# liuzhenboo/Stereo-Visual-Odometry

Hardware: AMD Instinct MI355X
Metric: stereo frames/sec on KITTI-00 1241x376; LK-kernel achieved HBM GB/s vs peak (higher is better)
Workload: dtype u8; 1 GPU; S0 synthetic KITTI-like stereo sequence 1241x376 (config #2 stand-in), FAST+LK track_mode LK_stereof2f_pnp, batched frame pairs (256 per step, 4 distinct chunks cycled), frames resident in HBM for `value`; `m1` (--full) = host-resident frames, H2D included; pairs_ok_last_step=256, parallelism=1 GPU

## Files before the change

stereo-visual-odometry_amd/binding.py:

```python
import ctypes as C
import os
import subprocess

import numpy as np

_HERE = os.path.dirname(os.path.abspath(__file__))
_LIB = None

MEM_HOST, MEM_DEVICE = 0, 1

KP_DTYPE = np.dtype([("x", "<f4"), ("y", "<f4"), ("size", "<f4"), ("angle", "<f4"),
                     ("response", "<f4"), ("octave", "<i4"), ("class_id", "<i4")])


class SvoError(RuntimeError):
    pass


class Config(C.Structure):
    _fields_ = [("width", C.c_int32), ("height", C.c_int32), ("max_keypoints", C.c_int32),
                ("max_batch", C.c_int32), ("num_slots", C.c_int32), ("fast_threshold", C.c_int32),
                ("num_features_tracking", C.c_int32), ("iterations", C.c_int32),
                ("reproj_err", C.c_float), ("confidence", C.c_float),
                ("feature_match_error", C.c_double), ("inlier_rate", C.c_double),
# ... 246 lines not shown
        return [(names[i].decode(), float(ms[i])) for i in range(n)]

    def _img(self, img, shape=None):
        shape = shape or (self.height, self.width)
        assert tuple(img.shape) == tuple(shape), (tuple(img.shape), shape)
        if isinstance(img, np.ndarray):
            assert img.dtype == np.uint8 and img.strides[1] == 1
            return C.c_void_p(img.ctypes.data), int(img.strides[0]), MEM_HOST
        assert img.element_size() == 1 and img.stride(1) == 1
        return C.c_void_p(img.data_ptr()), int(img.stride(0)), (MEM_DEVICE if img.is_cuda else MEM_HOST)

    def fast_detect(self, img, threshold=20, nonmax=True, cap=None):
        cap = cap or self.cfg.max_keypoints
        p, pitch, mem = self._img(img)
        out = np.zeros(cap, dtype=KP_DTYPE)
        n = C.c_int(0)
        self._check(self.lib.svo_fast_detect(self.h, p, pitch, mem, int(threshold), int(bool(nonmax)),
                                             C.c_void_p(out.ctypes.data), cap, C.byref(n)))
        return out[:n.value].copy()

    def build_pyramid(self, slot, img):
        p, pitch, mem = self._img(img)
        self._check(self.lib.svo_build_pyramid(self.h, int(slot), p, pitch, mem))

    def read_pyramid_level(self, slot, level):
        w, h = C.c_int(0), C.c_int(0)
        self._check(self.lib.svo_read_pyramid_level(self.h, slot, level, None, 0, MEM_HOST,
                                                    C.byref(w), C.byref(h)))
        out = np.zeros((h.value, w.value), np.uint8)
        self._check(self.lib.svo_read_pyramid_level(self.h, slot, level, C.c_void_p(out.ctypes.data),
                                                    w.value, MEM_HOST, C.byref(w), C.byref(h)))
        return out

    def lk_track(self, slot_prev, slot_next, pts):
        if isinstance(pts, np.ndarray):
            pts = np.ascontiguousarray(pts, np.float32).reshape(-1, 2)
            n = pts.shape[0]
            out = np.zeros((n, 2), np.float32)
            st = np.zeros(n, np.uint8)
        else:
            import torch
            n = pts.shape[0]
            out = torch.zeros((n, 2), dtype=torch.float32, device=pts.device)
            st = torch.zeros(n, dtype=torch.uint8, device=pts.device)
            self._order_in(st)
        pi, mem = _ptr(pts)
        po, _ = _ptr(out)
        ps, _ = _ptr(st)
        self._check(self.lib.svo_lk_track(self.h, slot_prev, slot_next, pi, n, po, ps, mem))
        if mem == MEM_DEVICE:
            self._order_out(st)
        return out, st

    def circular_match(self, slots, t1_left):
        if isinstance(t1_left, np.ndarray):
            t1_left = np.ascontiguousarray(t1_left, np.float32).reshape(-1, 2)
            n = t1_left.shape[0]
            outs = [np.zeros((max(n, 1), 2), np.float32) for _ in range(4)]
        else:
            import torch
            n = t1_left.shape[0]
            outs = [torch.zeros((max(n, 1), 2), dtype=torch.float32, device=t1_left.device) for _ in range(4)]
            self._order_in(outs[0])
        pi, mem = _ptr(t1_left)
        m = C.c_int(0)
        self._check(self.lib.svo_circular_match(self.h, *[int(s) for s in slots], pi, n,
# ... 374 lines not shown
```

stereo-visual-odometry_amd/csrc/fast.hip:

```cpp
#include "svo_device.h"
#include "svo_kernels.h"

namespace svo {

constexpr int kTileW = 64, kTileH = 16, kHalo = 4;
constexpr int kRawW = kTileW + 2 * kHalo;
constexpr int kRawH = kTileH + 2 * kHalo;
constexpr int kScW = kTileW + 2;
constexpr int kScH = kTileH + 2;

__device__ __forceinline__ void load_circle(const uint8_t *c, int d[16], int v)
{
    constexpr int P = kRawW;
    d[0] = v - c[3 * P];       d[1] = v - c[3 * P + 1];   d[2] = v - c[2 * P + 2];   d[3] = v - c[P + 3];
    d[4] = v - c[3];           d[5] = v - c[-P + 3];      d[6] = v - c[-2 * P + 2];  d[7] = v - c[-3 * P + 1];
    d[8] = v - c[-3 * P];      d[9] = v - c[-3 * P - 1];  d[10] = v - c[-2 * P - 2]; d[11] = v - c[-P - 3];
    d[12] = v - c[-3];         d[13] = v - c[P - 3];      d[14] = v - c[2 * P - 2];  d[15] = v - c[3 * P - 1];
}

__device__ __forceinline__ bool has_arc9(unsigned m16)
{
    unsigned m = m16 | (m16 << 16);
    unsigned a = m & (m >> 1);
    unsigned b = a & (a >> 2);
    unsigned c = b & (b >> 4);
    unsigned e = c & (m >> 8);
    return (e & 0xFFFFu) != 0;
}

__device__ __forceinline__ bool fast_arc(const uint8_t *c, int thr)
{
    int d[16];
    load_circle(c, d, c[0]);
    unsigned dark = 0, bright = 0;
#pragma unroll
    for (int k = 0; k < 16; k++) {
        dark |= (unsigned)(d[k] > thr) << k;
        bright |= (unsigned)(d[k] < -thr) << k;
// ... 112 lines not shown
            if (c0 + c1 + c2 + c3) {
                int base = 0;
                if (lane == 0) base = atomicAdd(&n_cand, c0 + c1 + c2 + c3);
                base = __builtin_amdgcn_readfirstlane(base);
                const int pos = sy * kScW + sxb;
                if (m4 & 1u) cand[base + __popcll(b0 & lt)] = (uint16_t)pos;
                if (m4 & 2u) cand[base + c0 + __popcll(b1 & lt)] = (uint16_t)(pos + 1);
                if (m4 & 4u) cand[base + c0 + c1 + __popcll(b2 & lt)] = (uint16_t)(pos + 2);
                if (m4 & 8u) cand[base + c0 + c1 + c2 + __popcll(b3 & lt)] = (uint16_t)(pos + 3);
            }
        }
    }
    __syncthreads();
    const int nc = n_cand;
    for (int i0 = 0; i0 < nc; i0 += 256) {
        const int i = i0 + tid;
        const int pos = i < nc ? cand[i] : 0;
        const int sy = pos / kScW, sx = pos - sy * kScW;
        const bool corner = i < nc && fast_arc(&raw[(sy + kHalo - 1) * kRawW + sx + kHalo - 1], a.thr);
        if (a.nms) list_push(corner, pos, corners, &n_corner);
        else if (corner) sc[pos] = 1;
    }
    __syncthreads();
    if (a.nms) {
        const int nk = n_corner;
        for (int i = tid; i < nk; i += 256) {
            const int pos = corners[i];
            const int sy = pos / kScW, sx = pos - sy * kScW;
            sc[pos] = (uint8_t)fast_corner_score(&raw[(sy + kHalo - 1) * kRawW + sx + kHalo - 1], a.thr);
        }
        __syncthreads();
    }

#pragma unroll
    for (int j = 0; j < kTileH / 4; j++) {
        int ly = threadIdx.y + 4 * j, lx = threadIdx.x;
        int gx = x0 + lx, gy = y0 + ly;
        const uint8_t *p = &sc[(ly + 1) * kScW + lx + 1];
        int s = p[0];
        if (a.nms && s) {
            bool keep = s > p[-1] && s > p[1] && s > p[-kScW - 1] && s > p[-kScW] && s > p[-kScW + 1] &&
                        s > p[kScW - 1] && s > p[kScW] && s > p[kScW + 1];
            if (!keep) s = 0;
        }
        bool inimg = gx < a.w && gy < a.h;
        if (!inimg) s = 0;
        unsigned long long m = __ballot(s != 0);
        if (inimg) score[(int64_t)gy * a.spitch + gx] = (uint8_t)s;
        if (threadIdx.x == 0 && m && gy < a.h) atomicAdd(&rowcount[gy], __popcll(m));
    }
}

__global__ __launch_bounds__(256) void fast_emit_kernel(FastArgs a)
{
    const int b = blockIdx.y;
    const int y = blockIdx.x * 4 + (threadIdx.x >> 6);
    const int lane = threadIdx.x & 63;
    if (y >= a.h) return;
    const uint8_t *score = a.score + (int64_t)b * a.score_stride + (int64_t)y * a.spitch;
    const int *rowcount = a.rowcount + (int64_t)b * a.rowcount_stride;
    int mine = rowcount[y];
    bool last = (y == a.h - 1);
    if (mine == 0 && !last) return;
    int part = 0;
    for (int r = lane; r < y; r += 64) part += rowcount[r];
    int off = wave_sum_i32(part);
    if (last && lane == 0) a.n_out[b] = off + mine;
    if (mine == 0) return;
    float2 *xy = a.kp_xy + (int64_t)b * a.kp_stride;
    float *resp = a.kp_resp + (int64_t)b * a.kp_stride;
    for (int x = lane; x < ((a.w + 63) & ~63); x += 64) {
        int s = x < a.w ? score[x] : 0;
        unsigned long long m = __ballot(s != 0);
        if (s) {
            int idx = off + __popcll(m & ((1ull << lane) - 1ull));
            if (idx < a.cap) {
                xy[idx] = make_float2((float)x, (float)y);
                resp[idx] = a.nms ? (float)s : 0.f;
            }
        }
        off += __popcll(m);
    }
}

__global__ __launch_bounds__(1024) void fast_keep_strongest_kernel(FastArgs a, int keep)
{
    __shared__ int hist[256];
    __shared__ int wave_eq[16], wave_kp[16];
    __shared__ int s_t, s_need_eq, s_eq_base, s_out_base;
    const int b = blockIdx.x, tid = threadIdx.x, lane = tid & 63, wv = tid >> 6;
    const int n = a.n_out[b];
    if (n <= keep || n > a.cap) return;
    float2 *xy = a.kp_xy + (int64_t)b * a.kp_stride;
    float *resp = a.kp_resp + (int64_t)b * a.kp_stride;
    if (tid < 256) hist[tid] = 0;
    __syncthreads();
    for (int i = tid; i < n; i += 1024) atomicAdd(&hist[min(255, max(0, (int)resp[i]))], 1);
    __syncthreads();
    if (tid == 0) {
        int above = 0, t = 255;
        for (; t > 0; t--) {
            if (above + hist[t] >= keep) break;
            above += hist[t];
        }
        s_t = t; s_need_eq = keep - above; s_eq_base = 0; s_out_base = 0;
    }
    __syncthreads();
    const int t = s_t, need_eq = s_need_eq;
    for (int start = 0; start < n; start += 1024) {
        const int i = start + tid;
        const bool in = i < n;
        const float2 p = in ? xy[i] : make_float2(0.f, 0.f);
        const float r = in ? resp[i] : 0.f;
        const int ri = (int)r;
// ... 178 lines not shown
```

stereo-visual-odometry_amd/csrc/pipeline.hip:

```cpp
#include <cstring>
#include "svo_ctx.h"

namespace svo {

void timing_mark(svo_ctx *ctx, const char *name)
{
    if (!ctx->timing) return;
    if (ctx->ev_used >= 16384) return;
    if (ctx->ev_used == ctx->ev_pool.size()) {
        hipEvent_t ev = nullptr;
        if (hipEventCreate(&ev) != hipSuccess) return;
        ctx->ev_pool.push_back(ev);
    }
    hipEvent_t ev = ctx->ev_pool[ctx->ev_used++];
    (void)hipEventRecord(ev, ctx->stream);
    ctx->marks.emplace_back(name, ev);
}
static inline void mark(svo_ctx *ctx, const char *name) { timing_mark(ctx, name); }

static const char *kTMatch = "orb_match";
static const char *kT0 = "start", *kTPyr = "pyramid", *kTFast = "fast", *kTLk = "lk", *kTCompact = "compact",
                  *kTTri = "triangulate", *kTPnp = "pnp", *kTFin = "finalize";

static int ingest_frames(svo_ctx *ctx, const uint8_t *L, const uint8_t *R, int pitch, int64_t frame_stride,
// ... 138 lines not shown

static int run_pairs(svo_ctx *ctx, int n_pairs, int fp0, int fc0, int fstep, const double *pose0_host,
                     svo_step_result *results_dev, const StreamStep *ss = nullptr)
{
    const PyrGeom &g = ctx->geom;
    const int cap = ctx->cfg.max_keypoints;
    if (ctx->cfg.track_mode == SVO_MODE_ORB) {
        if (ctx->back_pending) {
            SVO_HIP(hipStreamWaitEvent(ctx->stream, ctx->ev_back, 0));
            ctx->back_pending = false;
        }
        orb_match_pairs(ctx, n_pairs, fp0, fc0, fstep, ctx->stream);
        mark(ctx, kTMatch);
        const SnapSpec snap{(const int *)ctx->orb_n, (const int *)ctx->orb_overflow, fp0, fc0, fstep, 2};
        launch_triangulate_batch(ctx, n_pairs, cap, ctx->cmp[0], ctx->cmp[1], ctx->m_out, 0, &snap);
        mark(ctx, kTTri);
        return run_back(ctx, n_pairs, pose0_host, results_dev, false, ss);
    }
    auto S = [&](int slot) { return ctx->bslots + (size_t)slot * g.slot_bytes; };
    LkArgs a{};
    a.g = g; a.ncalls = 4;
    a.slot_stride = (int64_t)fstep * 2 * g.slot_bytes;
    a.prev[0] = S(2 * fp0);     a.next[0] = S(2 * fp0 + 1);
    a.prev[1] = S(2 * fp0 + 1); a.next[1] = S(2 * fc0 + 1);
    a.prev[2] = S(2 * fc0 + 1); a.next[2] = S(2 * fc0);
    a.prev[3] = S(2 * fc0);     a.next[3] = S(2 * fp0);
    a.pts_in = ctx->kp_xy + (size_t)fp0 * cap; a.pts_stride = (int64_t)fstep * cap;
    a.n_pts = ctx->kp_n + fp0;
    a.n_fixed = 0; a.cap = cap;
    for (int i = 0; i < 4; i++) { a.pts_out[i] = ctx->pts_out[i]; a.status[i] = ctx->status[i]; }
    a.keep = ctx->keep;
    a.match_err = ctx->cfg.feature_match_error; a.match_err_f = (float)ctx->cfg.feature_match_error;
    a.accum = ctx->cfg.lk_accum;
    launch_lk(a, n_pairs, cap, ctx->stream);
    mark(ctx, kTLk);
    if (ctx->back_pending) {
        SVO_HIP(hipStreamWaitEvent(ctx->stream, ctx->ev_back, 0));
        ctx->back_pending = false;
    }
    CompactArgs c{};
    c.keep = ctx->keep; c.n_pts = ctx->kp_n + fp0; c.n_fixed = 0; c.pts_stride = (int64_t)fstep * cap; c.cap = cap;
    c.in[0] = a.pts_in; c.in[1] = ctx->pts_out[0]; c.in[2] = ctx->pts_out[1]; c.in[3] = ctx->pts_out[2];
    for (int i = 0; i < 4; i++) c.out[i] = ctx->cmp[i];
    c.m_out = ctx->m_out;
    launch_compact(c, n_pairs, ctx->stream);
    mark(ctx, kTCompact);
    const SnapSpec snap{ctx->kp_n, nullptr, fp0, fc0, fstep, 1};
    static const bool tri_side = !(getenv("SVO_TRI_SIDE") && getenv("SVO_TRI_SIDE")[0] == '0');
    if (tri_side && ctx->overlap && results_dev != nullptr && !ss) {
        launch_snap_counts(ctx, n_pairs, snap, ctx->stream);
        mark(ctx, kTTri);
        return run_back(ctx, n_pairs, pose0_host, results_dev,  true);
    }
    launch_triangulate_batch(ctx, n_pairs, cap, ctx->cmp[0], ctx->cmp[1], ctx->m_out, 0, &snap);
    mark(ctx, kTTri);
    return run_back(ctx, n_pairs, pose0_host, results_dev, false, ss);
}

static int run_back(svo_ctx *ctx, int n_pairs, const double *pose0_host, svo_step_result *results_dev, bool triangulate_first,
                    const StreamStep *ss)
{
    hipStream_t bs = ctx->stream;
    const bool side = ctx->overlap && results_dev != nullptr && !ss;
    if (side) {
        SVO_HIP(hipEventRecord(ctx->ev_front, ctx->stream));
        SVO_HIP(hipStreamWaitEvent(ctx->side_stream, ctx->ev_front, 0));
        bs = ctx->side_stream;
    }
    if (triangulate_first)
        launch_triangulate_batch(ctx, n_pairs, ctx->cfg.max_keypoints, ctx->cmp[0], ctx->cmp[1], ctx->m_out, 0, nullptr, bs);
    launch_pnp_batch(ctx, n_pairs, ctx->cmp[3], ctx->m_out, 0, bs);
    if (!side) mark(ctx, kTPnp);
    const int *ovf = ctx->cfg.track_mode == SVO_MODE_ORB ? ctx->kp_n_snap + 2 * n_pairs : nullptr;
    if (ss) {
        for_stream_chunks(ss->ids, ss->init, n_pairs, [&](const StreamTable &tab, int i0, int n) {
            launch_finalize_streams(ctx, i0, n, n_pairs, ctx->kp_n_snap, ctx->kp_n_snap + n_pairs, ovf, tab, bs);
        });
    } else {
        launch_finalize_chain(ctx, n_pairs, ctx->kp_n_snap, ctx->kp_n_snap + n_pairs, ovf, pose0_host, bs);
    }
    const int rc = deliver_records(ctx, ctx->d_results, n_pairs, results_dev, SVO_MEM_DEVICE, bs);
    if (rc) return rc;
    if (side) {
        SVO_HIP(hipEventRecord(ctx->ev_back, ctx->side_stream));
        ctx->back_pending = true;
    } else {
        mark(ctx, kTFin);
    }
    return SVO_OK;
}

int deliver_records(svo_ctx *ctx, const svo_step_result *d_src, int n, svo_step_result *out, int mem, hipStream_t st)
{
    const size_t bytes = sizeof(svo_step_result) * (size_t)n;
    if (mem == SVO_MEM_DEVICE) {
        if (out) SVO_HIP(hipMemcpyAsync(out, d_src, bytes, hipMemcpyDeviceToDevice, st));
        return SVO_OK;
    }
    void *h = (char *)ctx->h_pinned + kPinnedRecords;
    SVO_HIP(hipMemcpyAsync(h, d_src, bytes, hipMemcpyDeviceToHost, st));
    SVO_HIP(hipStreamSynchronize(st));
    memcpy(out, h, bytes);
    return SVO_OK;
}
// ... 179 lines not shown
```

stereo-visual-odometry_amd/csrc/pyramid.hip:

```cpp
#include "svo_device.h"
#include "svo_kernels.h"

namespace svo {

__device__ __forceinline__ const uint8_t *src_image(const PyrArgs &a, int b)
{
    if (a.img2) return ((b & 1) ? a.img2 : a.img) + (int64_t)(b >> 1) * a.img_stride;
    return a.img + (int64_t)b * a.img_stride;
}

__global__ __launch_bounds__(256) void pyr_copy0_kernel(PyrArgs a)
{
    const int b = blockIdx.z, y = blockIdx.y * blockDim.y + threadIdx.y;
    const int w = a.g.w[0];
    if (y >= a.g.h[0]) return;
    const uint8_t *src = src_image(a, b) + (int64_t)y * a.pitch;
    uint8_t *dst = a.slots + (int64_t)b * a.slot_stride + a.g.origin[0] + (int64_t)y * a.g.pitch[0];
    const int x = (blockIdx.x * blockDim.x + threadIdx.x) * 16;
    if (x >= w) return;
    if (x + 16 <= w && ((uintptr_t)(src + x) & 15) == 0) {
        *(uint4 *)(dst + x) = *(const uint4 *)(src + x);
    } else {
        for (int q = 0; q < 16 && x + q < w; q++) dst[x + q] = src[x + q];
    }
}

constexpr int kBorderRows = 16;
constexpr int kFrameRowsPerWg = 4, kSidePasses = 4;
__host__ __device__ inline int border_top_groups() { return 2 * kPad / kFrameRowsPerWg; }
__host__ __device__ inline int border_side_groups(int h) { return (h + kBorderRows * kSidePasses - 1) / (kBorderRows * kSidePasses); }
__global__ __launch_bounds__(256) void pyr_border_kernel(PyrArgs a, int l)
{
    const int b = blockIdx.y;
    const int w = a.g.w[l], h = a.g.h[l], pitch = a.g.pitch[l];
    uint8_t *lvl = a.slots + (int64_t)b * a.slot_stride + a.g.origin[l];
    if ((int)blockIdx.x < border_top_groups()) {
        for (int q = 0; q < kFrameRowsPerWg; q++) {
            const int gidx = blockIdx.x * kFrameRowsPerWg + q;
            const int py = gidx < kPad ? gidx - kPad : h + (gidx - kPad);
            const uint8_t *src = lvl + (int64_t)refl101(py, h) * pitch;
            uint8_t *dst = lvl + (int64_t)py * pitch;
            for (int px = ((int)threadIdx.x << 2) - kPad; px < w + kPad; px += 1024) {
                uint32_t v = 0;
                if (px >= 0 && px + 4 <= w) v = *(const uint32_t *)(src + px);
                else {
#pragma unroll
                    for (int k = 0; k < 4; k++) v |= (uint32_t)src[refl101(min(px + k, w + kPad - 1), w)] << (8 * k);
                }
                if (px + 4 <= w + kPad) *(uint32_t *)(dst + px) = v;
                else for (int k = 0; px + k < w + kPad; k++) dst[px + k] = (uint8_t)(v >> (8 * k));
            }
        }
        return;
    }
    const int sgroup = blockIdx.x - border_top_groups();
    if (w >= 2 * kPad) {
        static_assert(kBorderRows == 16 && kPad == 32, "256 threads = 16 rows x 16 dwords");
        typedef uint32_t u32_unaligned __attribute__((aligned(1)));
        const int k = threadIdx.x & 15, r = threadIdx.x >> 4;
        const int px = k < 8 ? -kPad + 4 * k : w + 4 * (k - 8);
        const int c0 = k < 8 ? kPad - 3 - 4 * k : w - 5 - 4 * (k - 8);
        for (int q = 0; q < kSidePasses; q++) {
            const int py = (sgroup * kSidePasses + q) * kBorderRows + r;
            if (py >= h) return;
            uint8_t *row = lvl + (int64_t)py * pitch;
            const uint32_t v = *(const u32_unaligned *)(row + c0);
            *(u32_unaligned *)(row + px) = __builtin_amdgcn_perm(0u, v, 0x00010203u);
        }
    } else {
        const int t = threadIdx.x & 63;
        const int px = t < kPad ? t - kPad : w + (t - kPad);
        const int sx = refl101(px, w);
        for (int q = 0; q < kSidePasses; q++)
            for (int r = threadIdx.x >> 6; r < kBorderRows; r += 4) {
                const int py = (sgroup * kSidePasses + q) * kBorderRows + r;
                if (py >= h) return;
                uint8_t *row = lvl + (int64_t)py * pitch;
                row[px] = row[sx];
            }
    }
}

__global__ __launch_bounds__(256) void pyr_down_kernel(PyrArgs a, int l)
{
    const int b = blockIdx.z, y = blockIdx.y * blockDim.y + threadIdx.y;
    const int w = a.g.w[l];
    if (y >= a.g.h[l]) return;
    const int sp = a.g.pitch[l - 1];
    uint8_t *slot = a.slots + (int64_t)b * a.slot_stride;
    const uint8_t *src = slot + a.g.origin[l - 1];
    uint8_t *dst = slot + a.g.origin[l] + (int64_t)y * a.g.pitch[l];
    const int x0 = (blockIdx.x * blockDim.x + threadIdx.x) * 4;
    if (x0 >= w) return;
    int acc[4] = {0, 0, 0, 0};
#pragma unroll
    for (int r = 0; r < 5; r++) {
        const uint32_t *row = (const uint32_t *)(src + (int64_t)(2 * y + r - 2) * sp + 2 * x0 - 4);
        const uint32_t d0 = row[0], d1 = row[1], d2 = row[2], d3 = row[3];
        int s[16];
#pragma unroll
        for (int j = 0; j < 4; j++) {
            s[j] = (d0 >> (8 * j)) & 255; s[4 + j] = (d1 >> (8 * j)) & 255;
            s[8 + j] = (d2 >> (8 * j)) & 255; s[12 + j] = (d3 >> (8 * j)) & 255;
        }
        const int wv = (r == 2) ? 6 : ((r == 1 || r == 3) ? 4 : 1);
#pragma unroll
        for (int q = 0; q < 4; q++) {
            const int c = 4 + 2 * q;
            const int hs = s[c] * 6 + (s[c - 1] + s[c + 1]) * 4 + s[c - 2] + s[c + 2];
            acc[q] += hs * wv;
        }
    }
    uint32_t out = 0;
#pragma unroll
    for (int q = 0; q < 4; q++) out |= (uint32_t)((acc[q] + 128) >> 8) << (8 * q);
    if (x0 + 4 <= w) *(uint32_t *)(dst + x0) = out;
    else for (int q = 0; x0 + q < w; q++) dst[x0 + q] = (uint8_t)(out >> (8 * q));
}

__global__ __launch_bounds__(256) void pyr_read_level_kernel(PyrGeom g, const uint8_t *slot, int l,
                                                              uint8_t *out, int out_pitch)
{
    int x = blockIdx.x * 256 + threadIdx.x, y = blockIdx.y;
    if (x >= g.w[l]) return;
    out[(int64_t)y * out_pitch + x] = slot[g.origin[l] + (int64_t)y * g.pitch[l] + x];
}

void launch_pyramid(const PyrArgs &a, int batch, hipStream_t st)
{
    dim3 blk(256, 1, 1);
    auto shape = [](int lanes_per_row, int rows, dim3 &grid, dim3 &block, int batch) {
        const int bx = lanes_per_row < 256 ? lanes_per_row : 256, by = 256 / bx;
        block = dim3(bx, by, 1);
        grid = dim3((lanes_per_row + bx - 1) / bx, (rows + by - 1) / by, batch);
    };
    {
        dim3 g, bk;
        shape((a.g.w[0] + 15) / 16, a.g.h[0], g, bk, batch);
        hipLaunchKernelGGL(pyr_copy0_kernel, g, bk, 0, st, a);
    }
    for (int l = 0; l < a.g.nlevels; l++) {
        if (l > 0) {
            dim3 g, bk;
            shape((a.g.w[l] + 3) / 4, a.g.h[l], g, bk, batch);
            hipLaunchKernelGGL(pyr_down_kernel, g, bk, 0, st, a, l);
        }
        dim3 gb(border_top_groups() + border_side_groups(a.g.h[l]), batch, 1);
        hipLaunchKernelGGL(pyr_border_kernel, gb, blk, 0, st, a, l);
    }
}

void launch_pyr_read_level(const PyrGeom &g, const uint8_t *slot, int l, uint8_t *out, int out_pitch,
                           hipStream_t st)
{
    dim3 grid((g.w[l] + 255) / 256, g.h[l], 1), blk(256, 1, 1);
    hipLaunchKernelGGL(pyr_read_level_kernel, grid, blk, 0, st, g, slot, l, out, out_pitch);
}

}
```

stereo-visual-odometry_amd/csrc/svo_abi.hip:

```cpp
#include <cmath>
#include <cstdio>
#include <cstring>
#include <ctime>
#include <new>
#include <vector>
#include "svo_ctx.h"

using namespace svo;

static int align_up(int v, int a) { return (v + a - 1) / a * a; }

namespace svo {
int dev_alloc_raw(svo_ctx *ctx, void **out, size_t bytes)
{
    *out = nullptr;
    if (bytes == 0) bytes = 1;
    if (ctx->arena.planning) {
        ctx->arena.plan.emplace_back(out, ctx->arena.planned);
        ctx->arena.planned += (bytes + 255) / 256 * 256;
        return SVO_OK;
    }
    SVO_HIP(hipMalloc(out, bytes));
    ctx->arena.extra.push_back(*out);
    return SVO_OK;
// ... 71 lines not shown
    cfg->fast_threshold = 20;
    cfg->num_features_tracking = 5;
    cfg->iterations = 500;
    cfg->reproj_err = 0.5f;
    cfg->confidence = 0.99f;
    cfg->feature_match_error = 3.0;
    cfg->inlier_rate = 0.01;
    cfg->min_move2 = 0.0005 * 0.0005;
    cfg->max_move2 = 100.0;
    const double fx = 718.856, fy = 718.856, cx = 607.193, cy = 185.216, tx = -0.537;
    const double P1[12] = {fx, 0, cx, 0, 0, fy, cy, 0, 0, 0, 1, 0};
    const double P2[12] = {fx, 0, cx, fx * tx, 0, fy, cy, 0, 0, 0, 1, 0};
    memcpy(cfg->P1, P1, sizeof(P1));
    memcpy(cfg->P2, P2, sizeof(P2));
    cfg->track_mode = SVO_MODE_LK;
    cfg->orb_nfeatures = 2000;
    cfg->orb_scale_factor = 1.2f;
    cfg->orb_nlevels = 8;
    cfg->orb_ini_th = 20;
    cfg->orb_min_th = 7;
    cfg->fast_keep_strongest = 0;
    cfg->lk_accum = SVO_LK_ACCUM_EXACT;
}

static void free_all(svo_ctx *c)
{
    dev_release(c);
    for (int k = 0; k < 2; k++) if (c->resize_scratch[k]) (void)hipFree(c->resize_scratch[k]);
    if (c->ingest.src_stage) (void)hipFree(c->ingest.src_stage);
    if (c->bucket_cells) (void)hipFree(c->bucket_cells);
    if (c->bucket_stage) (void)hipFree(c->bucket_stage);
    if (c->ev_front) (void)hipEventDestroy(c->ev_front);
    if (c->ev_back) (void)hipEventDestroy(c->ev_back);
    if (c->ev_order) (void)hipEventDestroy(c->ev_order);
    if (c->side_stream) (void)hipStreamDestroy(c->side_stream);
    for (int k = 0; k < 2; k++) {
        if (c->ev_up[k]) (void)hipEventDestroy(c->ev_up[k]);
        if (c->ev_fb_free[k]) (void)hipEventDestroy(c->ev_fb_free[k]);
    }
    if (c->copy_stream) (void)hipStreamDestroy(c->copy_stream);
    for (int k = 0; k < 2; k++)
        if (c->ev_async[k]) (void)hipEventDestroy(c->ev_async[k]);
    if (c->fetch_stream) (void)hipStreamDestroy(c->fetch_stream);
    if (c->h_pinned) (void)hipHostFree(c->h_pinned);
    if (c->h_stage) (void)hipHostFree(c->h_stage);
    for (int k = 0; k < 2; k++) if (c->ev_stage[k]) (void)hipEventDestroy(c->ev_stage[k]);
    for (auto &e : c->ev_pool) (void)hipEventDestroy(e);
    if (c->own_stream) (void)hipStreamDestroy(c->own_stream);
}

static double now_ms()
{
    timespec ts;
    clock_gettime(CLOCK_MONOTONIC, &ts);
    return ts.tv_sec * 1e3 + ts.tv_nsec * 1e-6;
}
#define PHASE(name) do { if (timing_on) { const double t__ = now_ms(); fprintf(stderr, "[svo_create] %8.2f ms  %s\n", t__ - t_phase, name); t_phase = t__; } } while (0)

extern "C" int svo_create(const svo_config *cfg, int device, svo_ctx **out)
{
    if (!cfg || !out) return SVO_ERR_ARG;
    const bool timing_on = getenv("SVO_TIMING") != nullptr;
    double t_phase = now_ms();
    *out = nullptr;
    if (cfg->width < 32 || cfg->height < 32 || cfg->max_keypoints < 64 || cfg->max_batch < 1 ||
        cfg->num_slots < 4 || cfg->width > 16384 || cfg->height > 16384)
// ... 55 lines not shown
        DA(ctx->pts_out[i], sizeof(float2) * (size_t)cap * B_lk);
        DA(ctx->status[i], (size_t)cap * B_lk);
        DA(ctx->cmp[i], sizeof(float2) * (size_t)cap * B);
    }
    DA(ctx->keep, (size_t)cap * B_lk);
    DA(ctx->m_out, sizeof(int) * (size_t)B);
    DA(ctx->X3, sizeof(float) * 3 * (size_t)cap * B);
    if (geom_workspace_bytes(*cfg, B, &ctx->pnp_ws_bytes) != SVO_OK) return fail(SVO_ERR_ARG);
    PHASE("plan + kernel attributes (code object load)");
    DA(ctx->pnp_ws, ctx->pnp_ws_bytes);
    dev_defer(ctx, [ctx]() { return geom_workspace_init(ctx); });
    DA(ctx->d_results, sizeof(svo_step_result) * (size_t)B);
    DA(ctx->bslots, orb ? 256 : (size_t)2 * n_img * ctx->geom.slot_bytes);
    DA(ctx->kp_n_snap, sizeof(int) * (size_t)(3 * n_img));
    if (B > 1) {
        const size_t per_cam = (size_t)ctx->stage_pitch * h * (size_t)(B + 1);
        for (int k = 0; k < 2; k++) {
            DA(ctx->fb[k], 2 * per_cam);
            DA(ctx->d_async[k], sizeof(svo_step_result) * (size_t)B);
        }
    }
    if (orb) {
        int rc = orb_alloc(ctx);
        if (rc != SVO_OK) { fprintf(stderr, "svo_create: %s\n", ctx->err.c_str()); return fail(rc); }
    }
#undef DA
    if (dev_commit(ctx) != SVO_OK) { fprintf(stderr, "svo_create: device memory (%zu MB): %s\n", ctx->arena.planned >> 20, ctx->err.c_str()); return fail(SVO_ERR_HIP); }
    PHASE("one device allocation + deferred initialisation");
    CK(hipHostMalloc(&ctx->h_stage, (size_t)ctx->stage_pitch * h * 2, hipHostMallocDefault));
    for (int k = 0; k < 2; k++) CK(hipEventCreateWithFlags(&ctx->ev_stage[k], hipEventDisableTiming));
    CK(hipStreamCreateWithFlags(&ctx->side_stream, hipStreamNonBlocking));
    CK(hipEventCreateWithFlags(&ctx->ev_front, hipEventDisableTiming));
    CK(hipEventCreateWithFlags(&ctx->ev_back, hipEventDisableTiming));
    if (B > 1) {
        for (int k = 0; k < 2; k++) {
            CK(hipEventCreateWithFlags(&ctx->ev_up[k], hipEventDisableTiming));
            CK(hipEventCreateWithFlags(&ctx->ev_fb_free[k], hipEventDisableTiming));
            CK(hipEventCreateWithFlags(&ctx->ev_async[k], hipEventDisableTiming));
        }
        CK(hipStreamCreateWithFlags(&ctx->copy_stream, hipStreamNonBlocking));
        CK(hipStreamCreateWithFlags(&ctx->fetch_stream, hipStreamNonBlocking));
        ctx->async_ready = true;
    }
    ctx->h_pinned_bytes = kPinnedRecords + sizeof(svo_step_result) * (size_t)B +
                          (size_t)cap * (sizeof(svo_keypoint) + 32) + sizeof(int) * 64;
    CK(hipHostMalloc(&ctx->h_pinned, ctx->h_pinned_bytes, hipHostMallocDefault));
    PHASE("events, streams, page-locked scratch");
    CK(hipStreamSynchronize(ctx->stream));
    PHASE("stream sync");
#undef CK
    *out = ctx;
    return SVO_OK;
}

extern "C" void svo_destroy(svo_ctx *ctx)
{
    if (!ctx) return;
    (void)hipSetDevice(ctx->device);
    if (ctx->stream) (void)hipStreamSynchronize(ctx->stream);
    if (ctx->side_stream) (void)hipStreamSynchronize(ctx->side_stream);
    free_all(ctx);
    delete ctx;
}

extern "C" const char *svo_last_error(const svo_ctx *ctx) { return ctx ? ctx->err.c_str() : "null context"; }

// ... 167 lines not shown
    int rc = resolve_image(ctx, img, pitch, mem, 0, &d, &dp);
    if (rc) return rc;
    PyrArgs a{};
    a.g = ctx->geom; a.img = d; a.pitch = dp; a.img_stride = 0;
    a.slots = ctx->slots + (size_t)slot * ctx->geom.slot_bytes; a.slot_stride = 0;
    launch_pyramid(a, 1, ctx->stream);
    SVO_HIP(hipGetLastError());
    if (mem == SVO_MEM_HOST) SVO_HIP(hipStreamSynchronize(ctx->stream));
    ctx->slot_built[slot] = 1;
    return SVO_OK;
}

extern "C" int svo_read_pyramid_level(svo_ctx *ctx, int slot, int level, uint8_t *out, int out_pitch,
                                      int mem, int *w, int *h)
{
    if (!ctx) return SVO_ERR_ARG;
    SVO_ARG(slot >= 0 && slot < ctx->cfg.num_slots, "slot out of range");
    SVO_ARG(level >= 0 && level < ctx->geom.nlevels, "level out of range");
    if (!ctx->slot_built[slot]) { ctx->err = "pyramid slot not built"; return SVO_ERR_STATE; }
    const int lw = ctx->geom.w[level], lh = ctx->geom.h[level];
    if (w) *w = lw;
    if (h) *h = lh;
    if (!out) return SVO_OK;
    SVO_ARG(out_pitch >= lw, "out_pitch < level width");
    SVO_HIP(hipSetDevice(ctx->device));
    const uint8_t *s = ctx->slots + (size_t)slot * ctx->geom.slot_bytes;
    if (mem == SVO_MEM_DEVICE) {
        launch_pyr_read_level(ctx->geom, s, level, out, out_pitch, ctx->stream);
        SVO_HIP(hipGetLastError());
        return SVO_OK;
    }
    SVO_HIP(hipMemcpy2DAsync(out, out_pitch, s + ctx->geom.origin[level], ctx->geom.pitch[level], lw, lh,
                             hipMemcpyDeviceToHost, ctx->stream));
    SVO_HIP(hipStreamSynchronize(ctx->stream));
    return SVO_OK;
}

template <typename T>
static int to_device(svo_ctx *ctx, const T *src, T *scratch, int n, int mem, const T **d)
{
    if (mem == SVO_MEM_DEVICE) { *d = src; return SVO_OK; }
    SVO_HIP(hipMemcpyAsync(scratch, src, sizeof(T) * (size_t)n, hipMemcpyHostToDevice, ctx->stream));
    *d = scratch;
    return SVO_OK;
}

static void fill_lk_common(svo_ctx *ctx, LkArgs &a, int n)
{
    a.g = ctx->geom;
    a.slot_stride = 0;
    a.pts_stride = 0;
    a.n_pts = nullptr; a.n_fixed = n; a.cap = n;
    a.match_err = ctx->cfg.feature_match_error;
    a.match_err_f = (float)ctx->cfg.feature_match_error;
    a.accum = ctx->cfg.lk_accum;
}

extern "C" int svo_lk_track(svo_ctx *ctx, int slot_prev, int slot_next, const svo_pt2f *prev_pts, int n,
                            svo_pt2f *next_pts, uint8_t *status, int mem)
{
    if (!ctx) return SVO_ERR_ARG;
    SVO_ARG(slot_prev >= 0 && slot_prev < ctx->cfg.num_slots && slot_next >= 0 &&
            slot_next < ctx->cfg.num_slots, "slot out of range");
    SVO_ARG(n >= 0 && n <= ctx->cfg.max_keypoints, "n exceeds max_keypoints");
    SVO_ARG(mem == SVO_MEM_HOST || mem == SVO_MEM_DEVICE, "bad mem");
    if (!ctx->slot_built[slot_prev] || !ctx->slot_built[slot_next]) { ctx->err = "pyramid slot not built"; return SVO_ERR_STATE; }
// ... 865 lines not shown
```

stereo-visual-odometry_amd/csrc/svo_ctx.h:

```cpp
#pragma once
#include <hip/hip_runtime.h>
#include <functional>
#include <string>
#include <utility>
#include <vector>
#include "../../include/svo_abi.h"
#include "svo_kernels.h"

struct DevArena {
    char *base = nullptr;
    size_t planned = 0;
    bool planning = false;
    std::vector<std::pair<void **, size_t>> plan;
    std::vector<std::function<int()>> after;
    std::vector<void *> extra;
};

struct StreamSet {
    int n = 0;
    int n_seg = 0;
    uint8_t *seg[4] = {nullptr, nullptr, nullptr, nullptr};
    size_t seg_bytes[4] = {0, 0, 0, 0};
    double *pose = nullptr;
    std::vector<int> n_frames;
// ... 59 lines not shown
    bool orb_ready = false;
    bool orb_qt_parallel = false;
    bool orb_level0_in_slot = false;
    bool orb_resize_staged = false;
    bool orb_copy_level0 = false;
    svo::OrbGeom orb_geom;
    uint8_t *orb_slots = nullptr, *orb_blur = nullptr;
    void *orb_xtab = nullptr, *orb_ytab = nullptr;
    float4 *orb_cell_cand = nullptr; int *orb_cell_cnt = nullptr;
    float4 *orb_lvl_cand = nullptr; int *orb_lvl_cnt = nullptr;
    int orb_node_cap = 0;
    void *orb_qkeys = nullptr, *orb_qtmp = nullptr;
    int *orb_sel = nullptr, *orb_sel_cnt = nullptr, *orb_overflow = nullptr;
    void *orb_kps = nullptr; uint8_t *orb_desc = nullptr; int *orb_n = nullptr; int orb_kp_cap = 0, orb_cand_cap = 0;
    int *orb_midx[2] = {nullptr, nullptr}; float *orb_mdist[2] = {nullptr, nullptr};
    void *h_pinned = nullptr; size_t h_pinned_bytes = 0;
    bool overlap = false;
    hipStream_t side_stream = nullptr;
    uint8_t *fb[2] = {nullptr, nullptr};
    hipStream_t copy_stream = nullptr;
    hipEvent_t ev_up[2] = {nullptr, nullptr}, ev_fb_free[2] = {nullptr, nullptr};
    bool fb_used[2] = {false, false};
    int fb_frames[2] = {0, 0};
    int fb_first[2] = {0, 0};
    svo_step_result *d_async[2] = {nullptr, nullptr};
    hipEvent_t ev_async[2] = {nullptr, nullptr};
    int async_n[2] = {0, 0};
    unsigned async_head = 0, async_tail = 0;
    int async_last_pairs = 0;
    const double *seed_dev = nullptr;
    hipStream_t fetch_stream = nullptr;
    bool async_ready = false;
    hipEvent_t ev_front = nullptr, ev_back = nullptr;
    hipEvent_t ev_order = nullptr;
    bool back_pending = false;
    int *kp_n_snap = nullptr;
    StreamSet streams;
    std::vector<ResizeTab> resize_tabs;
    uint8_t *resize_scratch[2] = {nullptr, nullptr};
    size_t resize_scratch_bytes[2] = {0, 0};
    Ingest ingest;
    int bucket_w = 0, bucket_h = 0, bucket_keep = 0;
    int *bucket_cells = nullptr;
    size_t bucket_cells_bytes = 0;
    uint8_t *bucket_stage = nullptr;
    size_t bucket_stage_bytes = 0;
    bool timing = false;
    std::vector<hipEvent_t> ev_pool;
    size_t ev_used = 0;
    std::vector<std::pair<const char *, hipEvent_t>> marks;
    std::vector<std::pair<const char *, float>> last_times;
};

#define SVO_HIP(call)                                                                         \
    do {                                                                                      \
        hipError_t e__ = (call);                                                              \
        if (e__ != hipSuccess) {                                                              \
            ctx->err = std::string(#call) + ": " + hipGetErrorString(e__);                    \
            return SVO_ERR_HIP;                                                               \
        }                                                                                     \
    } while (0)

#define SVO_ARG(cond, msg)                                                                    \
    do {                                                                                      \
        if (!(cond)) { ctx->err = std::string("bad argument: ") + msg; return SVO_ERR_ARG; }   \
    } while (0)
// ... 50 lines not shown
```

Measured before the change: 17910 stereo pairs/s.

## Fuse pyramid border fill into level kernels and vectorize FAST score and emit

The pyramid build now stages rows in LDS and writes reflected borders in the same kernel, replacing the separate copy and border-fill launches. Small levels get a per-pixel fallback path. FAST uses taller tiles and writes scores four bytes at a time using row-wide sums, and the emit kernel scans 16 bytes per lane with a wave prefix scan. The LK launch now waits on a new solver event from the side stream when enough pairs are pending, which adds a dependency that may reduce overlap. A debug readback for padded pyramids is also added.

```diff
diff --git a/stereo-visual-odometry_amd/binding.py b/stereo-visual-odometry_amd/binding.py
--- a/stereo-visual-odometry_amd/binding.py
+++ b/stereo-visual-odometry_amd/binding.py
@@ -302,6 +302,16 @@
                                                     w.value, MEM_HOST, C.byref(w), C.byref(h)))
         return out
 
+    def debug_read_pyramid_padded(self, slot, level, batch=False):
+        w, h = self.width, self.height
+        for _ in range(level):
+            w, h = (w + 1) // 2, (h + 1) // 2
+        fn = self.lib.svo_debug_read_pyramid_padded
+        fn.argtypes = [C.c_void_p, C.c_int, C.c_int, C.c_void_p, C.c_int]
+        out = np.zeros((h + 64, w + 64), np.uint8)
+        self._check(fn(self.h, int(slot), int(level), C.c_void_p(out.ctypes.data), int(bool(batch))))
+        return out
+
     def lk_track(self, slot_prev, slot_next, pts):
         if isinstance(pts, np.ndarray):
             pts = np.ascontiguousarray(pts, np.float32).reshape(-1, 2)
diff --git a/stereo-visual-odometry_amd/csrc/fast.hip b/stereo-visual-odometry_amd/csrc/fast.hip
--- a/stereo-visual-odometry_amd/csrc/fast.hip
+++ b/stereo-visual-odometry_amd/csrc/fast.hip
@@ -3,7 +3,7 @@
 
 namespace svo {
 
-constexpr int kTileW = 64, kTileH = 16, kHalo = 4;
+constexpr int kTileW = 64, kTileH = 32, kHalo = 4;
 constexpr int kRawW = kTileW + 2 * kHalo;
 constexpr int kRawH = kTileH + 2 * kHalo;
 constexpr int kScW = kTileW + 2;
@@ -182,22 +182,36 @@
         __syncthreads();
     }
 
-#pragma unroll
-    for (int j = 0; j < kTileH / 4; j++) {
-        int ly = threadIdx.y + 4 * j, lx = threadIdx.x;
-        int gx = x0 + lx, gy = y0 + ly;
-        const uint8_t *p = &sc[(ly + 1) * kScW + lx + 1];
-        int s = p[0];
-        if (a.nms && s) {
-            bool keep = s > p[-1] && s > p[1] && s > p[-kScW - 1] && s > p[-kScW] && s > p[-kScW + 1] &&
-                        s > p[kScW - 1] && s > p[kScW] && s > p[kScW + 1];
-            if (!keep) s = 0;
-        }
-        bool inimg = gx < a.w && gy < a.h;
-        if (!inimg) s = 0;
-        unsigned long long m = __ballot(s != 0);
-        if (inimg) score[(int64_t)gy * a.spitch + gx] = (uint8_t)s;
-        if (threadIdx.x == 0 && m && gy < a.h) atomicAdd(&rowcount[gy], __popcll(m));
+    static_assert((kTileH * (kTileW / 4)) % 256 == 0, "whole trips: the row sums run with every lane");
+    for (int i = tid; i < kTileH * (kTileW / 4); i += 256) {
+        const int ly = i >> 4, lq = i & 15;
+        const int gx = x0 + 4 * lq, gy = y0 + ly;
+        uint8_t n[3][6];
+#pragma unroll
+        for (int r = 0; r < 3; r++)
+#pragma unroll
+            for (int c = 0; c < 6; c++) n[r][c] = sc[(ly + r) * kScW + 4 * lq + c];
+        uint32_t out = 0;
+        int cnt = 0;
+#pragma unroll
+        for (int q = 0; q < 4; q++) {
+            int s = n[1][q + 1];
+            if (a.nms) {
+                const bool keep = s > n[1][q] && s > n[1][q + 2] && s > n[0][q] && s > n[0][q + 1] && s > n[0][q + 2] &&
+                                  s > n[2][q] && s > n[2][q + 1] && s > n[2][q + 2];
+                if (!keep) s = 0;
+            }
+            if (gx + q >= a.w || gy >= a.h) s = 0;
+            out |= (uint32_t)s << (8 * q);
+            cnt += s != 0;
+        }
+        const int rowsum = row_allsum_i32(cnt);
+        if (gy < a.h) {
+            uint8_t *dst = score + (int64_t)gy * a.spitch + gx;
+            if (gx + 4 <= a.w) *(uint32_t *)dst = out;
+            else for (int q = 0; gx + q < a.w; q++) dst[q] = (uint8_t)(out >> (8 * q));
+            if (lq == 0 && rowsum) atomicAdd(&rowcount[gy], rowsum);
+        }
     }
 }
 
@@ -219,17 +233,28 @@
     if (mine == 0) return;
     float2 *xy = a.kp_xy + (int64_t)b * a.kp_stride;
     float *resp = a.kp_resp + (int64_t)b * a.kp_stride;
-    for (int x = lane; x < ((a.w + 63) & ~63); x += 64) {
-        int s = x < a.w ? score[x] : 0;
-        unsigned long long m = __ballot(s != 0);
-        if (s) {
-            int idx = off + __popcll(m & ((1ull << lane) - 1ull));
+    for (int xb = 0; xb < a.w; xb += 16 * 64) {
+        const int x = xb + 16 * lane;
+        uint4 v = make_uint4(0u, 0u, 0u, 0u);
+        if (x < a.w) v = *(const uint4 *)(score + x);
+        const uint32_t d[4] = {v.x, v.y, v.z, v.w};
+        unsigned m = 0;
+#pragma unroll
+        for (int k = 0; k < 16; k++) m |= (unsigned)(((d[k >> 2] >> (8 * (k & 3))) & 255u) != 0 && x + k < a.w) << k;
+        const int cnt = __popc(m);
+        const int incl = wave_incl_scan(cnt);
+        int idx = off + incl - cnt;
+        off += __builtin_amdgcn_readlane(incl, 63);
+        while (m) {
+            const int k = __ffs(m) - 1;
+            m &= m - 1;
             if (idx < a.cap) {
-                xy[idx] = make_float2((float)x, (float)y);
-                resp[idx] = a.nms ? (float)s : 0.f;
+                const uint32_t dk = k < 8 ? (k < 4 ? v.x : v.y) : (k < 12 ? v.z : v.w);
+                xy[idx] = make_float2((float)(x + k), (float)y);
+                resp[idx] = a.nms ? (float)((dk >> (8 * (k & 3))) & 255u) : 0.f;
             }
-        }
-        off += __popcll(m);
+            idx++;
+        }
     }
 }
 
diff --git a/stereo-visual-odometry_amd/csrc/pipeline.hip b/stereo-visual-odometry_amd/csrc/pipeline.hip
--- a/stereo-visual-odometry_amd/csrc/pipeline.hip
+++ b/stereo-visual-odometry_amd/csrc/pipeline.hip
@@ -194,6 +194,8 @@
     a.keep = ctx->keep;
     a.match_err = ctx->cfg.feature_match_error; a.match_err_f = (float)ctx->cfg.feature_match_error;
     a.accum = ctx->cfg.lk_accum;
+    constexpr int kLkWaitPairs = 64;
+    if (ctx->back_pending && n_pairs >= kLkWaitPairs) SVO_HIP(hipStreamWaitEvent(ctx->stream, ctx->ev_solver, 0));
     launch_lk(a, n_pairs, cap, ctx->stream);
     mark(ctx, kTLk);
     if (ctx->back_pending) {
@@ -232,6 +234,7 @@
     if (triangulate_first)
         launch_triangulate_batch(ctx, n_pairs, ctx->cfg.max_keypoints, ctx->cmp[0], ctx->cmp[1], ctx->m_out, 0, nullptr, bs);
     launch_pnp_batch(ctx, n_pairs, ctx->cmp[3], ctx->m_out, 0, bs);
+    if (side) SVO_HIP(hipEventRecord(ctx->ev_solver, ctx->side_stream));
     if (!side) mark(ctx, kTPnp);
     const int *ovf = ctx->cfg.track_mode == SVO_MODE_ORB ? ctx->kp_n_snap + 2 * n_pairs : nullptr;
     if (ss) {
diff --git a/stereo-visual-odometry_amd/csrc/pyramid.hip b/stereo-visual-odometry_amd/csrc/pyramid.hip
--- a/stereo-visual-odometry_amd/csrc/pyramid.hip
+++ b/stereo-visual-odometry_amd/csrc/pyramid.hip
@@ -9,113 +9,144 @@
     return a.img + (int64_t)b * a.img_stride;
 }
 
-__global__ __launch_bounds__(256) void pyr_copy0_kernel(PyrArgs a)
+__host__ __device__ inline bool pyr_small_level(int w, int h) { return w <= kPad + 1 || h <= kPad + 1; }
+__host__ __device__ inline int pyr_row_bytes(int w) { return (w + 2 * kPad + 15) & ~15; }
+
+__device__ inline int pyr_down_pixel(const uint8_t *src, int sp, int x, int y)
 {
-    const int b = blockIdx.z, y = blockIdx.y * blockDim.y + threadIdx.y;
-    const int w = a.g.w[0];
-    if (y >= a.g.h[0]) return;
-    const uint8_t *src = src_image(a, b) + (int64_t)y * a.pitch;
-    uint8_t *dst = a.slots + (int64_t)b * a.slot_stride + a.g.origin[0] + (int64_t)y * a.g.pitch[0];
-    const int x = (blockIdx.x * blockDim.x + threadIdx.x) * 16;
-    if (x >= w) return;
-    if (x + 16 <= w && ((uintptr_t)(src + x) & 15) == 0) {
-        *(uint4 *)(dst + x) = *(const uint4 *)(src + x);
-    } else {
-        for (int q = 0; q < 16 && x + q < w; q++) dst[x + q] = src[x + q];
+    int acc = 0;
+#pragma unroll
+    for (int r = 0; r < 5; r++) {
+        const uint8_t *row = src + (int64_t)(2 * y + r - 2) * sp + 2 * x;
+        const int wv = (r == 2) ? 6 : ((r == 1 || r == 3) ? 4 : 1);
+        acc += (row[0] * 6 + (row[-1] + row[1]) * 4 + row[-2] + row[2]) * wv;
+    }
+    return (acc + 128) >> 8;
+}
+
+template <bool kLevel0>
+__device__ inline void pyr_small_level_bytes(const PyrArgs &a, int l, int b)
+{
+    const int w = a.g.w[l], h = a.g.h[l], pw = w + 2 * kPad, ph = h + 2 * kPad;
+    uint8_t *slot = a.slots + (int64_t)b * a.slot_stride;
+    uint8_t *lvl = slot + a.g.origin[l];
+    const int nthr = blockDim.x * blockDim.y, tid = threadIdx.y * blockDim.x + threadIdx.x;
+    for (int i = blockIdx.x * nthr + tid; i < pw * ph; i += gridDim.x * nthr) {
+        const int py = i / pw - kPad, px = i - (py + kPad) * pw - kPad;
+        const int sx = refl101(px, w), sy = refl101(py, h);
+        int v;
+        if (kLevel0) v = src_image(a, b)[(int64_t)sy * a.pitch + sx];
+        else v = pyr_down_pixel(slot + a.g.origin[l - 1], a.g.pitch[l - 1], sx, sy);
+        lvl[(int64_t)py * a.g.pitch[l] + px] = (uint8_t)v;
     }
 }
 
-constexpr int kBorderRows = 16;
-constexpr int kFrameRowsPerWg = 4, kSidePasses = 4;
-__host__ __device__ inline int border_top_groups() { return 2 * kPad / kFrameRowsPerWg; }
-__host__ __device__ inline int border_side_groups(int h) { return (h + kBorderRows * kSidePasses - 1) / (kBorderRows * kSidePasses); }
-__global__ __launch_bounds__(256) void pyr_border_kernel(PyrArgs a, int l)
+template <int K, typename T>
+__device__ __forceinline__ void pyr_load_rows(const uint8_t *src, int pitch, uint8_t *lds, int P, int w, int y0, int h)
 {
-    const int b = blockIdx.y;
-    const int w = a.g.w[l], h = a.g.h[l], pitch = a.g.pitch[l];
-    uint8_t *lvl = a.slots + (int64_t)b * a.slot_stride + a.g.origin[l];
-    if ((int)blockIdx.x < border_top_groups()) {
-        for (int q = 0; q < kFrameRowsPerWg; q++) {
-            const int gidx = blockIdx.x * kFrameRowsPerWg + q;
-            const int py = gidx < kPad ? gidx - kPad : h + (gidx - kPad);
-            const uint8_t *src = lvl + (int64_t)refl101(py, h) * pitch;
-            uint8_t *dst = lvl + (int64_t)py * pitch;
-            for (int px = ((int)threadIdx.x << 2) - kPad; px < w + kPad; px += 1024) {
-                uint32_t v = 0;
-                if (px >= 0 && px + 4 <= w) v = *(const uint32_t *)(src + px);
-                else {
+    constexpr int S = (int)sizeof(T);
+    for (int c = threadIdx.x; c * S < w; c += blockDim.x) {
+        const bool full = (c + 1) * S <= w;
+        T v[K];
 #pragma unroll
-                    for (int k = 0; k < 4; k++) v |= (uint32_t)src[refl101(min(px + k, w + kPad - 1), w)] << (8 * k);
-                }
-                if (px + 4 <= w + kPad) *(uint32_t *)(dst + px) = v;
-                else for (int k = 0; px + k < w + kPad; k++) dst[px + k] = (uint8_t)(v >> (8 * k));
-            }
+        for (int k = 0; k < K; k++) {
+            const int j = threadIdx.y + k * blockDim.y;
+            v[k] = *(const T *)(src + (int64_t)min(y0 + j, h - 1) * pitch + (full ? c * S : 0));
         }
-        return;
-    }
-    const int sgroup = blockIdx.x - border_top_groups();
-    if (w >= 2 * kPad) {
-        static_assert(kBorderRows == 16 && kPad == 32, "256 threads = 16 rows x 16 dwords");
-        typedef uint32_t u32_unaligned __attribute__((aligned(1)));
-        const int k = threadIdx.x & 15, r = threadIdx.x >> 4;
-        const int px = k < 8 ? -kPad + 4 * k : w + 4 * (k - 8);
-        const int c0 = k < 8 ? kPad - 3 - 4 * k : w - 5 - 4 * (k - 8);
-        for (int q = 0; q < kSidePasses; q++) {
-            const int py = (sgroup * kSidePasses + q) * kBorderRows + r;
-            if (py >= h) return;
-            uint8_t *row = lvl + (int64_t)py * pitch;
-            const uint32_t v = *(const u32_unaligned *)(row + c0);
-            *(u32_unaligned *)(row + px) = __builtin_amdgcn_perm(0u, v, 0x00010203u);
+#pragma unroll
+        for (int k = 0; k < K; k++) {
+            const int j = threadIdx.y + k * blockDim.y;
+            uint8_t *row = lds + j * P + kPad;
+            if (full && y0 + j < h) *(T *)(row + c * S) = v[k];
+            if (!full && y0 + j < h)
+                for (int q = c * S; q < w; q++) row[q] = src[(int64_t)(y0 + j) * pitch + q];
         }
-    } else {
-        const int t = threadIdx.x & 63;
-        const int px = t < kPad ? t - kPad : w + (t - kPad);
-        const int sx = refl101(px, w);
-        for (int q = 0; q < kSidePasses; q++)
-            for (int r = threadIdx.x >> 6; r < kBorderRows; r += 4) {
-                const int py = (sgroup * kSidePasses + q) * kBorderRows + r;
-                if (py >= h) return;
-                uint8_t *row = lvl + (int64_t)py * pitch;
-                row[px] = row[sx];
-            }
     }
 }
 
+template <int K>
+__device__ __forceinline__ void pyr_emit_rows(uint8_t *lvl, int pitch, uint8_t *lds, int P, int w, int h, int y0)
+{
+    __syncthreads();
+#pragma unroll
+    for (int k = 0; k < K; k++) {
+        const int j = threadIdx.y + k * blockDim.y;
+        if (y0 + j >= h) continue;
+        uint8_t *row = lds + j * P;
+        for (int t = threadIdx.x; t < 2 * kPad + 16; t += blockDim.x) {
+            if (t < kPad) row[t] = row[2 * kPad - t];
+            else if (t < 2 * kPad) row[w + t] = row[w + 2 * kPad - 2 - t];
+            else if (w + t < P) row[w + t] = 0;
+        }
+    }
+    __syncthreads();
+    for (int c = threadIdx.x; c * 16 < P; c += blockDim.x) {
+#pragma unroll
+        for (int k = 0; k < K; k++) {
+            const int j = threadIdx.y + k * blockDim.y, y = y0 + j;
+            if (y >= h) continue;
+            const uint4 v = *(const uint4 *)(lds + j * P + c * 16);
+            uint8_t *col = lvl - kPad + c * 16;
+            *(uint4 *)(col + (int64_t)y * pitch) = v;
+            if (y >= 1 && y <= kPad) *(uint4 *)(col - (int64_t)y * pitch) = v;
+            if (y >= h - 1 - kPad && y <= h - 2) *(uint4 *)(col + (int64_t)(2 * (h - 1) - y) * pitch) = v;
+        }
+    }
+}
+
+template <int K>
+__global__ __launch_bounds__(256) void pyr_level0_kernel(PyrArgs a)
+{
+    extern __shared__ uint4 pyr_lds[];
+    const int b = blockIdx.y, w = a.g.w[0], h = a.g.h[0];
+    if (pyr_small_level(w, h)) { pyr_small_level_bytes<true>(a, 0, b); return; }
+    uint8_t *lds = (uint8_t *)pyr_lds;
+    const int P = pyr_row_bytes(w), y0 = blockIdx.x * K * blockDim.y;
+    const uint8_t *src = src_image(a, b);
+    const unsigned al = (unsigned)(uintptr_t)src | (unsigned)a.pitch;
+    if ((al & 15) == 0) pyr_load_rows<K, uint4>(src, a.pitch, lds, P, w, y0, h);
+    else if ((al & 3) == 0) pyr_load_rows<K, uint32_t>(src, a.pitch, lds, P, w, y0, h);
+    else pyr_load_rows<K, uint8_t>(src, a.pitch, lds, P, w, y0, h);
+    pyr_emit_rows<K>(a.slots + (int64_t)b * a.slot_stride + a.g.origin[0], a.g.pitch[0], lds, P, w, h, y0);
+}
+
+template <int K>
 __global__ __launch_bounds__(256) void pyr_down_kernel(PyrArgs a, int l)
 {
-    const int b = blockIdx.z, y = blockIdx.y * blockDim.y + threadIdx.y;
-    const int w = a.g.w[l];
-    if (y >= a.g.h[l]) return;
+    extern __shared__ uint4 pyr_lds[];
+    const int b = blockIdx.y, w = a.g.w[l], h = a.g.h[l];
+    if (pyr_small_level(w, h)) { pyr_small_level_bytes<false>(a, l, b); return; }
+    uint8_t *lds = (uint8_t *)pyr_lds;
+    const int P = pyr_row_bytes(w), y0 = blockIdx.x * K * blockDim.y;
     const int sp = a.g.pitch[l - 1];
     uint8_t *slot = a.slots + (int64_t)b * a.slot_stride;
     const uint8_t *src = slot + a.g.origin[l - 1];
-    uint8_t *dst = slot + a.g.origin[l] + (int64_t)y * a.g.pitch[l];
-    const int x0 = (blockIdx.x * blockDim.x + threadIdx.x) * 4;
-    if (x0 >= w) return;
-    int acc[4] = {0, 0, 0, 0};
+    constexpr int NR = 2 * K + 3;
+    const int jb = threadIdx.y * K, yb = y0 + jb;
+    for (int x0 = threadIdx.x * 4; x0 < w && yb < h; x0 += blockDim.x * 4) {
+        uint32_t hs[NR][4];
 #pragma unroll
-    for (int r = 0; r < 5; r++) {
-        const uint32_t *row = (const uint32_t *)(src + (int64_t)(2 * y + r - 2) * sp + 2 * x0 - 4);
-        const uint32_t d0 = row[0], d1 = row[1], d2 = row[2], d3 = row[3];
-        int s[16];
+        for (int r = 0; r < NR; r++) {
+            const uint32_t *row = (const uint32_t *)(src + (int64_t)(2 * yb + r - 2) * sp + 2 * x0 - 4);
+            const uint32_t d0 = row[0], d1 = row[1], d2 = row[2], d3 = row[3];
+            const uint32_t W[6] = {__builtin_amdgcn_alignbyte(d1, d0, 2), d1, __builtin_amdgcn_alignbyte(d2, d1, 2), d2,
+                                   __builtin_amdgcn_alignbyte(d3, d2, 2), d3};
 #pragma unroll
-        for (int j = 0; j < 4; j++) {
-            s[j] = (d0 >> (8 * j)) & 255; s[4 + j] = (d1 >> (8 * j)) & 255;
-            s[8 + j] = (d2 >> (8 * j)) & 255; s[12 + j] = (d3 >> (8 * j)) & 255;
+            for (int q = 0; q < 4; q++)
+                hs[r][q] = __builtin_amdgcn_udot4(W[q + 2], 0x00000001u, __builtin_amdgcn_udot4(W[q], 0x04060401u, 0u, false), false);
         }
-        const int wv = (r == 2) ? 6 : ((r == 1 || r == 3) ? 4 : 1);
 #pragma unroll
-        for (int q = 0; q < 4; q++) {
-            const int c = 4 + 2 * q;
-            const int hs = s[c] * 6 + (s[c - 1] + s[c + 1]) * 4 + s[c - 2] + s[c + 2];
-            acc[q] += hs * wv;
+        for (int k = 0; k < K; k++) {
+            uint32_t out = 0;
+#pragma unroll
+            for (int q = 0; q < 4; q++) {
+                const uint32_t v = hs[2 * k][q] + hs[2 * k + 4][q] + 4 * (hs[2 * k + 1][q] + hs[2 * k + 3][q]) + 6 * hs[2 * k + 2][q];
+                out |= ((v + 128) >> 8) << (8 * q);
+            }
+            if (yb + k < h) *(uint32_t *)(lds + (jb + k) * P + kPad + x0) = out;
         }
     }
-    uint32_t out = 0;
-#pragma unroll
-    for (int q = 0; q < 4; q++) out |= (uint32_t)((acc[q] + 128) >> 8) << (8 * q);
-    if (x0 + 4 <= w) *(uint32_t *)(dst + x0) = out;
-    else for (int q = 0; x0 + q < w; q++) dst[x0 + q] = (uint8_t)(out >> (8 * q));
+    pyr_emit_rows<K>(slot + a.g.origin[l], a.g.pitch[l], lds, P, w, h, y0);
 }
 
 __global__ __launch_bounds__(256) void pyr_read_level_kernel(PyrGeom g, const uint8_t *slot, int l,
@@ -128,25 +159,24 @@
 
 void launch_pyramid(const PyrArgs &a, int batch, hipStream_t st)
 {
-    dim3 blk(256, 1, 1);
-    auto shape = [](int lanes_per_row, int rows, dim3 &grid, dim3 &block, int batch) {
-        const int bx = lanes_per_row < 256 ? lanes_per_row : 256, by = 256 / bx;
-        block = dim3(bx, by, 1);
-        grid = dim3((lanes_per_row + bx - 1) / bx, (rows + by - 1) / by, batch);
-    };
-    {
-        dim3 g, bk;
-        shape((a.g.w[0] + 15) / 16, a.g.h[0], g, bk, batch);
-        hipLaunchKernelGGL(pyr_copy0_kernel, g, bk, 0, st, a);
-    }
+    constexpr int kRows = 2;
     for (int l = 0; l < a.g.nlevels; l++) {
-        if (l > 0) {
-            dim3 g, bk;
-            shape((a.g.w[l] + 3) / 4, a.g.h[l], g, bk, batch);
-            hipLaunchKernelGGL(pyr_down_kernel, g, bk, 0, st, a, l);
+        const int w = a.g.w[l], h = a.g.h[l];
+        dim3 grid, block;
+        size_t lds = 0;
+        if (pyr_small_level(w, h)) {
+            grid = dim3(((w + 2 * kPad) * (h + 2 * kPad) + 255) / 256, batch, 1);
+            block = dim3(256, 1, 1);
+        } else {
+            const int P = pyr_row_bytes(w);
+            const int lanes = l == 0 ? P / 16 : (w + 3) / 4;
+            const int bx = lanes < 256 ? lanes : 256, by = 256 / bx, rows = kRows * by;
+            grid = dim3((h + rows - 1) / rows, batch, 1);
+            block = dim3(bx, by, 1);
+            lds = (size_t)rows * P;
         }
-        dim3 gb(border_top_groups() + border_side_groups(a.g.h[l]), batch, 1);
-        hipLaunchKernelGGL(pyr_border_kernel, gb, blk, 0, st, a, l);
+        if (l == 0) hipLaunchKernelGGL(pyr_level0_kernel<kRows>, grid, block, lds, st, a);
+        else hipLaunchKernelGGL(pyr_down_kernel<kRows>, grid, block, lds, st, a, l);
     }
 }
 
diff --git a/stereo-visual-odometry_amd/csrc/svo_abi.hip b/stereo-visual-odometry_amd/csrc/svo_abi.hip
--- a/stereo-visual-odometry_amd/csrc/svo_abi.hip
+++ b/stereo-visual-odometry_amd/csrc/svo_abi.hip
@@ -127,6 +127,7 @@
     if (c->bucket_stage) (void)hipFree(c->bucket_stage);
     if (c->ev_front) (void)hipEventDestroy(c->ev_front);
     if (c->ev_back) (void)hipEventDestroy(c->ev_back);
+    if (c->ev_solver) (void)hipEventDestroy(c->ev_solver);
     if (c->ev_order) (void)hipEventDestroy(c->ev_order);
     if (c->side_stream) (void)hipStreamDestroy(c->side_stream);
     for (int k = 0; k < 2; k++) {
@@ -248,6 +249,7 @@
     CK(hipStreamCreateWithFlags(&ctx->side_stream, hipStreamNonBlocking));
     CK(hipEventCreateWithFlags(&ctx->ev_front, hipEventDisableTiming));
     CK(hipEventCreateWithFlags(&ctx->ev_back, hipEventDisableTiming));
+    CK(hipEventCreateWithFlags(&ctx->ev_solver, hipEventDisableTiming));
     if (B > 1) {
         for (int k = 0; k < 2; k++) {
             CK(hipEventCreateWithFlags(&ctx->ev_up[k], hipEventDisableTiming));
@@ -481,6 +483,28 @@
     }
     SVO_HIP(hipMemcpy2DAsync(out, out_pitch, s + ctx->geom.origin[level], ctx->geom.pitch[level], lw, lh,
                              hipMemcpyDeviceToHost, ctx->stream));
+    SVO_HIP(hipStreamSynchronize(ctx->stream));
+    return SVO_OK;
+}
+
+extern "C" int svo_debug_read_pyramid_padded(svo_ctx *ctx, int slot, int level, uint8_t *out, int batch)
+{
+    if (!ctx || !out) return SVO_ERR_ARG;
+    SVO_ARG(level >= 0 && level < ctx->geom.nlevels, "level out of range");
+    const uint8_t *base;
+    if (batch) {
+        SVO_ARG(ctx->cfg.track_mode == SVO_MODE_LK && slot >= 0 && slot < 2 * ctx->n_img, "batch slot out of range");
+        base = ctx->bslots;
+    } else {
+        SVO_ARG(slot >= 0 && slot < ctx->cfg.num_slots, "slot out of range");
+        if (!ctx->slot_built[slot]) { ctx->err = "pyramid slot not built"; return SVO_ERR_STATE; }
+        base = ctx->slots;
+    }
+    SVO_HIP(hipSetDevice(ctx->device));
+    const PyrGeom &g = ctx->geom;
+    const int pw = g.w[level] + 2 * kPad, ph = g.h[level] + 2 * kPad;
+    const uint8_t *s = base + (size_t)slot * g.slot_bytes + g.origin[level] - (int64_t)kPad * g.pitch[level] - kPad;
+    SVO_HIP(hipMemcpy2DAsync(out, pw, s, g.pitch[level], pw, ph, hipMemcpyDeviceToHost, ctx->stream));
     SVO_HIP(hipStreamSynchronize(ctx->stream));
     return SVO_OK;
 }
diff --git a/stereo-visual-odometry_amd/csrc/svo_ctx.h b/stereo-visual-odometry_amd/csrc/svo_ctx.h
--- a/stereo-visual-odometry_amd/csrc/svo_ctx.h
+++ b/stereo-visual-odometry_amd/csrc/svo_ctx.h
@@ -115,6 +115,7 @@
     hipStream_t fetch_stream = nullptr;
     bool async_ready = false;
     hipEvent_t ev_front = nullptr, ev_back = nullptr;
+    hipEvent_t ev_solver = nullptr;
     hipEvent_t ev_order = nullptr;
     bool back_pending = false;
     int *kp_n_snap = nullptr;
```

Measured after the change: 18030 stereo pairs/s (median of 6 runs). No clear change (+0.7%).
